# vovach777/llcomp

Hardware: AMD Instinct MI355X
Metric: encode+decode MPix/s on 4K RGB8, bit-exact (higher is better)
Workload: dtype int32

## Files before the change

llcomp_amd/csrc/dec_rows_asm.hpp:

```cpp
#pragma once
#include <cstdint>

namespace llcomp_mi {

#define LD_E0L "v32"
#define LD_E0H "v33"
#define LD_E0 "v[32:33]"
#define LD_E5L "v34"
#define LD_E5H "v35"
#define LD_E5 "v[34:35]"
#define LD_E6L "v36"
#define LD_E6H "v37"
#define LD_E6 "v[36:37]"
#define LD_E7L "v38"
#define LD_E7H "v39"
#define LD_E7 "v[38:39]"
#define LD_E1L "v40"
#define LD_E1H "v41"
#define LD_E1 "v[40:41]"
#define LD_E2L "v42"
#define LD_E2H "v43"
#define LD_E2 "v[42:43]"
#define LD_E3L "v44"
#define LD_E3H "v45"
#define LD_E3 "v[44:45]"
#define LD_E4L "v48"
#define LD_E4H "v49"
#define LD_E4 "v[48:49]"
#define LD_PROD "v50"
#define LD_R1 "v51"
#define LD_DIFF "v52"
#define LD_OFF "v52"
#define LD_EX "v32"
#define LD_W "v33"
#define LD_RUN "v40"
#define LD_NX "v41"
#define LD_T "v42"
#define LD_SX "s[56:57]"
#define LD_SA "s[58:59]"
#define LD_SW "s[60:61]"
#define LD_SP "s[62:63]"
#define LD_S5 "s[64:65]"
#define LD_SU "s[66:67]"
#define LD_SD "s[68:69]"
#define LD_S1L "s[68:69]"
#define LD_SM "s[70:71]"
#define LD_S1 "s70"
#define LD_S2 "s71"

#define LD_SPLIT(EL)                                                                                                       \
    "v_mul_u32_u24_sdwa " LD_PROD ", " EL ", %[range] dst_sel:DWORD dst_unused:UNUSED_PAD src0_sel:BYTE_1 src1_sel:DWORD\n\t" \
    "v_lshrrev_b32_e32 " LD_R1 ", 8, " LD_PROD "\n\t"                                                                      \
    "v_sub_u32_e32 %[range], %[range], " LD_R1 "\n\t"
#define LD_SPLIT_IN(EL)                                                                                                       \
    "v_mul_u32_u24_sdwa " LD_PROD ", " EL ", %[range_in] dst_sel:DWORD dst_unused:UNUSED_PAD src0_sel:BYTE_1 src1_sel:DWORD\n\t" \
    "v_lshrrev_b32_e32 " LD_R1 ", 8, " LD_PROD "\n\t"                                                                      \
    "v_sub_u32_e32 %[range], %[range_in], " LD_R1 "\n\t"
#define LD_REFILL(N)                                         \
    "v_cmp_gt_u32_e32 vcc, %[c100], %[range]\n\t"            \
    "s_and_saveexec_b64 " LD_SW ", vcc\n\t"                  \
    "s_cbranch_execz .Lrf" N "_%=\n\t"                       \
    "v_lshlrev_b32_e32 %[range], 8, %[range]\n\t"            \
    "v_perm_b32 %[low], %[low], %[w32], %[sel]\n\t"          \
    "v_lshrrev_b32_e32 %[w32], 8, %[w32]\n"                   \
    ".Lrf" N "_%=:\n\t"                                      \
    "s_mov_b64 exec, " LD_SW "\n\t"
#define LD_REFILL_R1(N)                                           \
    "v_cmp_gt_u32_e32 vcc, %[c100], " LD_R1 "\n\t"                \
    "s_and_saveexec_b64 " LD_SW ", vcc\n\t"                       \
    "s_cbranch_execz .Lrf" N "_%=\n\t"                            \
    "v_and_b32_e32 %[range], 0xffffff00, " LD_PROD "\n\t"         \
    "v_perm_b32 %[low], %[low], %[w32], %[sel]\n\t"               \
    "v_lshrrev_b32_e32 %[w32], 8, %[w32]\n"                        \
    ".Lrf" N "_%=:\n\t"                                           \
    "s_mov_b64 exec, " LD_SW "\n\t"
#define LD_UNARY(EL, EH, OFS, N, SAVE)                                      \
    LD_SPLIT(EL)                                                            \
    "v_sub_co_u32_e32 %[low], vcc, %[low], %[range]\n\t"                    \
    "ds_write_b16_d16_hi %[bank], " EL " offset:" OFS "\n\t"                \
    "s_andn2_b64 exec, exec, vcc\n\t"                                       \
    SAVE                                                                    \
    "s_cbranch_execz .Lx_done_%=\n\t"                                       \
    "ds_write_b16_d16_hi %[bank], " EH " offset:" OFS "\n\t"                \
    "v_add_u32_e32 " LD_EX ", 1, " LD_EX "\n\t"                                     \
    "v_mov_b32_e32 %[range], " LD_R1 "\n\t"                                 \
    LD_REFILL_R1(N)
#define LD_FETCH_REST                                         \
    "v_lshrrev_b32_e32 " LD_E1L ", 16, %[w0]\n\t"             \
    "v_and_b32_e32 " LD_E2L ", 0xffff, %[w1]\n\t"             \
    "v_lshrrev_b32_e32 " LD_E3L ", 16, %[w1]\n\t"             \
    "v_and_b32_e32 " LD_E4L ", 0xffff, %[w2]\n\t"             \
    "ds_read_b64 " LD_E1 ", " LD_E1L "\n\t"                   \
    "ds_read_b64 " LD_E2 ", " LD_E2L "\n\t"                   \
    "ds_read_b64 " LD_E3 ", " LD_E3L "\n\t"                   \
    "ds_read_b64 " LD_E4 ", " LD_E4L "\n\t"                   \
    "v_lshrrev_b32_e32 " LD_E5L ", 16, %[w2]\n\t"             \
    "v_and_b32_e32 " LD_E6L ", 0xffff, %[w3]\n\t"             \
    "v_lshrrev_b32_e32 " LD_E7L ", 16, %[w3]\n\t"             \
    "ds_read_b64 " LD_E5 ", " LD_E5L "\n\t"                   \
    "ds_read_b64 " LD_E6 ", " LD_E6L "\n\t"                   \
    "ds_read_b64 " LD_E7 ", " LD_E7L "\n\t"

__device__ __forceinline__ void dec_rows_sample_asm(uint32_t low_in, uint32_t range_in, unsigned long long win_in, uint32_t& low,
                                                    uint32_t& range, unsigned long long& win, uint32_t w0, uint32_t w1, uint32_t w2,
                                                    uint32_t w3, uint32_t bank, uint32_t& hot, uint32_t& value, uint32_t& w32) {
    asm volatile(
        "s_mov_b64 " LD_SX ", exec\n\t"
        "v_and_b32_e32 %[w32], 0xffffff, %[winl_in]\n\t"
        "v_or_b32_e32 %[w32], 0x1000000, %[w32]\n\t"
        "v_and_b32_e32 " LD_OFF ", 0xffff, %[w0]\n\t"
        "ds_read_b64 " LD_E0 ", " LD_OFF "\n\t"
        "v_mov_b32_e32 %[value], 0\n\t"
        "s_cmp_lg_u32 %[hot], 0\n\t"
        "s_cbranch_scc0 .Lcold_%=\n\t"
        LD_FETCH_REST
        "s_waitcnt lgkmcnt(7)\n\t"
        "s_branch .Lzero_%=\n"
        ".Lcold_%=:\n\t"
        "s_waitcnt lgkmcnt(0)\n"
        ".Lzero_%=:\n\t"
        LD_SPLIT_IN(LD_E0L)
        "v_sub_co_u32_e32 %[low], vcc, %[low_in], %[range]\n\t"
        "ds_write_b16_d16_hi %[bank], " LD_E0L "\n\t"
        "s_and_b64 " LD_SA ", exec, vcc\n\t"
        "v_cndmask_b32_e32 %[low], %[low], %[low_in], vcc\n\t"
        "s_andn2_b64 exec, exec, vcc\n\t"
        "s_cbranch_execz .Lz1_%=\n\t"
        "v_mov_b32_e32 %[range], " LD_R1 "\n\t"
        "ds_write_b16_d16_hi %[bank], " LD_E0H "\n"
        ".Lz1_%=:\n\t"
        "s_mov_b64 exec, " LD_SX "\n\t"
        LD_REFILL("0")
        "s_and_b64 exec, " LD_SA ", " LD_SA "\n\t"
        "s_cbranch_execz .Ldone_%=\n\t"
        "s_cmp_lg_u32 %[hot], 0\n\t"
        "s_cbranch_scc1 .Lhave_%=\n\t"
        LD_FETCH_REST
        ".Lhave_%=:\n\t"
        "v_mov_b32_e32 " LD_EX ", 0\n\t"
        "v_mov_b32_e32 " LD_W ", 1\n\t"
        "s_waitcnt lgkmcnt(0)\n\t"
        "s_mov_b64 " LD_SM ", 0\n\t"
        LD_UNARY(LD_E1L, LD_E1H, "2", "1", "s_mov_b64 " LD_S1L ", exec\n\t")
        LD_UNARY(LD_E2L, LD_E2H, "256", "2", "s_mov_b64 " LD_SM ", exec\n\t")
        LD_UNARY(LD_E3L, LD_E3H, "258", "3", "")
        "s_mov_b64 " LD_SU ", exec\n\t"
        ".p2align 6\n"
        ".Lu_%=:\n\t"
        "s_waitcnt lgkmcnt(0)\n\t"
        LD_SPLIT(LD_E4L)
        "v_sub_co_u32_e32 %[low], vcc, %[low], %[range]\n\t"
        "s_andn2_b64 exec, exec, vcc\n\t"
        "s_cbranch_execz .Lu_done_%=\n\t"
        "v_lshrrev_b32_e32 " LD_OFF ", 16, " LD_E4H "\n\t"
        "ds_read_b64 " LD_E4 ", " LD_OFF "\n\t"
        "v_add_u32_e32 " LD_EX ", 1, " LD_EX "\n\t"
        "v_mov_b32_e32 %[range], " LD_R1 "\n\t"
        LD_REFILL_R1("4")
        "s_branch .Lu_%=\n"
        ".Lu_done_%=:\n\t"
        "s_mov_b64 exec, " LD_SU "\n\t"
        "ds_write_b16_d16_hi %[bank], " LD_E4L " offset:512\n"
        ".Lx_done_%=:\n\t"
        "s_mov_b64 exec, " LD_SA "\n\t"
        "v_add_u32_e32 %[low], %[low], %[range]\n\t"
        LD_REFILL("5")
        "v_cmp_lt_u32_e32 vcc, 31, " LD_EX "\n\t"
        "s_cbranch_vccz .Lexok_%=\n\t"
        "s_and_saveexec_b64 " LD_SP ", vcc\n\t"
        "v_mov_b32_e32 %[w32], 0\n\t"
        "s_andn2_b64 exec, " LD_SP ", exec\n\t"
        "s_cbranch_execz .Ldone_%=\n"
        ".Lexok_%=:\n\t"
        "s_mov_b64 " LD_S5 ", exec\n\t"
        "s_and_b64 exec, exec, " LD_S1L "\n\t"
        "s_cbranch_execz .Lvalue_%=\n\t"
        "s_mov_b64 " LD_SU ", exec\n\t"
        LD_SPLIT(LD_E5L)
        "v_sub_co_u32_e32 " LD_DIFF ", vcc, %[low], %[range]\n\t"
        "ds_write_b16_d16_hi %[bank], " LD_E5L " offset:514\n\t"
        "s_andn2_b64 " LD_SP ", exec, vcc\n\t"
        "v_addc_co_u32_e32 " LD_W ", vcc, " LD_W ", " LD_W ", vcc\n\t"
        "v_mov_b32_e32 " LD_RUN ", 0\n\t"
        "s_and_b64 exec, " LD_SP ", " LD_SP "\n\t"
        "s_cbranch_execz .Lp5_%=\n\t"
        "v_mov_b32_e32 %[low], " LD_DIFF "\n\t"
        "v_mov_b32_e32 %[range], " LD_R1 "\n\t"
        "ds_write_b16_d16_hi %[bank], " LD_E5H " offset:514\n"
        ".Lp5_%=:\n\t"
        "s_mov_b64 exec, " LD_SU "\n\t"
        LD_REFILL("6")
        "v_add_u32_e32 " LD_T ", -1, " LD_EX "\n\t"
        "s_and_b64 exec, exec, " LD_SM "\n\t"
        "s_cbranch_execz .Lm_skip_%=\n\t"
        "s_mov_b64 " LD_SP ", exec\n\t"
        "v_add_u32_e32 " LD_NX ", -2, " LD_EX "\n\t"
        "v_lshrrev_b32_e32 " LD_RUN ", " LD_NX ", %[sentv]\n\t"
        ".p2align 6\n"
        ".Lm_%=:\n\t"
        "s_waitcnt lgkmcnt(0)\n\t"
        LD_SPLIT(LD_E6L)
        "v_sub_co_u32_e32 " LD_DIFF ", vcc, %[low], %[range]\n\t"
        "s_nop 1\n\t"
        "v_cndmask_b32_e32 %[range], " LD_R1 ", %[range], vcc\n\t"
        "v_cndmask_b32_e32 %[low], " LD_DIFF ", %[low], vcc\n\t"
        "v_cndmask_b32_e32 " LD_NX ", " LD_E6H ", " LD_E6L ", vcc\n\t"
        "v_addc_co_u32_e32 " LD_RUN ", vcc, " LD_RUN ", " LD_RUN ", vcc\n\t"
        "s_mov_b64 " LD_SD ", vcc\n\t"
        "v_lshrrev_b32_e32 " LD_OFF ", 16, " LD_NX "\n\t"
        "ds_read_b64 " LD_E6 ", " LD_OFF "\n\t"
        "v_cmp_gt_u32_e32 vcc, %[c100], %[range]\n\t"
        "s_and_saveexec_b64 " LD_SW ", vcc\n\t"
        "s_cbranch_execz .Lmr_%=\n\t"
        "v_lshlrev_b32_e32 %[range], 8, %[range]\n\t"
        "v_perm_b32 %[low], %[low], %[w32], %[sel]\n\t"
        "v_lshrrev_b32_e32 %[w32], 8, %[w32]\n"
        ".Lmr_%=:\n\t"
        "s_andn2_b64 exec, " LD_SW ", " LD_SD "\n\t"
        "s_cbranch_execnz .Lm_%=\n\t"
        "s_mov_b64 exec, " LD_SP "\n\t"
        "ds_write_b16_d16_hi %[bank], " LD_NX " offset:768\n"
        ".Lm_skip_%=:\n\t"
        "s_mov_b64 exec, " LD_SU "\n\t"
        "v_lshlrev_b32_e32 " LD_W ", " LD_T ", " LD_W "\n\t"
        "v_or_b32_e32 " LD_W ", " LD_W ", " LD_RUN "\n"
        ".Lvalue_%=:\n\t"
        "s_mov_b64 exec, " LD_S5 "\n\t"
        "v_lshlrev_b32_e64 " LD_T ", " LD_EX ", 1\n\t"
        "v_add_u32_e32 " LD_T ", -1, " LD_T "\n\t"
        "v_xor_b32_e32 %[value], " LD_W ", " LD_T "\n\t"
        LD_SPLIT(LD_E7L)
        "v_sub_co_u32_e32 " LD_DIFF ", vcc, %[low], %[range]\n\t"
        "ds_write_b16_d16_hi %[bank], " LD_E7L " offset:770\n\t"
        "s_andn2_b64 exec, exec, vcc\n\t"
        "s_cbranch_execz .Lp7_%=\n\t"
        "v_mov_b32_e32 %[low], " LD_DIFF "\n\t"
        "v_mov_b32_e32 %[range], " LD_R1 "\n\t"
        "ds_write_b16_d16_hi %[bank], " LD_E7H " offset:770\n\t"
        "v_sub_u32_e32 %[value], 0, %[value]\n"
        ".Lp7_%=:\n\t"
        "s_mov_b64 exec, " LD_S5 "\n\t"
        LD_REFILL("7")
        ".Ldone_%=:\n\t"
        "s_mov_b64 exec, " LD_SX "\n\t"
        "v_ffbh_u32_e32 " LD_DIFF ", %[w32]\n\t"
        "v_add_u32_e32 " LD_DIFF ", -7, " LD_DIFF "\n\t"
        "v_lshrrev_b64 %[win], " LD_DIFF ", %[win_in]\n\t"
        "s_bcnt1_i32_b64 " LD_S1 ", " LD_SA "\n\t"
        "s_bcnt1_i32_b64 " LD_S2 ", " LD_SX "\n\t"
        "s_lshl_b32 " LD_S1 ", " LD_S1 ", 1\n\t"
        "s_cmp_ge_u32 " LD_S1 ", " LD_S2 "\n\t"
        "s_cselect_b32 %[hot], 1, 0\n\t"
        "s_mov_b64 exec, " LD_SX "\n\t"
        : [low] "=&v"(low), [range] "=&v"(range), [win] "=&v"(win), [hot] "+s"(hot), [value] "=&v"(value), [w32] "=&v"(w32)
        : [low_in] "v"(low_in), [range_in] "v"(range_in), [win_in] "v"(win_in), [winl_in] "v"(uint32_t(win_in)), [w0] "v"(w0), [w1] "v"(w1), [w2] "v"(w2), [w3] "v"(w3), [bank] "v"(bank), [c100] "s"(0x100u), [sel] "s"(0x06050400u),
          [sentv] "v"(0x80000000u)
        : "vcc", "scc", "memory", "v32", "v33", "v34", "v35", "v36", "v37", "v38", "v39", "v40", "v41", "v42", "v43", "v44", "v45",
          "v48", "v49", "v50", "v51", "v52", "s56", "s57", "s58", "s59", "s60", "s61", "s62", "s63", "s64", "s65", "s66",
          "s67", "s68", "s69", "s70", "s71");
}

}
```

llcomp_amd/csrc/slice_kernels.hip:

```cpp
#include <algorithm>
#include <type_traits>

#include "device_common.hpp"
#include "kernels.hpp"

#ifndef LLMI_ASM_ENC
#define LLMI_ASM_ENC 1
#endif
#if LLMI_ASM_ENC
#include "enc_rows_asm.hpp"
#endif
#ifndef LLMI_ASM_DEC
#define LLMI_ASM_DEC 1
#endif
#if LLMI_ASM_DEC
#include "dec_rows_asm.hpp"
#endif

namespace llcomp_mi {

namespace {

#ifdef LLMI_CLOCK_PROBE
constexpr uint32_t kProbeSlots = 1u << 15;
// ... 839 lines not shown
        "v_cndmask_b32_e32 %[nx], %[hi], %[lo], vcc\n\t"
        "v_addc_co_u32_e32 %[w], vcc, %[w], %[w], vcc"
        : [diff] "=&v"(diff), [range] "=&v"(d.range), [low] "+v"(d.low), [nx] "=&v"(nx), [w] "+v"(w)
        : [r0] "v"(r0), [r1] "v"(r1), [lo] "v"(uint32_t(cur)), [hi] "v"(uint32_t(cur >> 32))
        : "vcc");
    if (d.range < 0x100) {
        d.range <<= 8;
        d.low = (d.low << 8) | (uint32_t(d.win) & 0xFF);
        d.win = window_next(d.win);
    }
    return nx;
}
template <int SLOT, bool CHECKED, bool INLDS>
__device__ __forceinline__ bool dec_once(RangeDec& d, Bank& bank, const Entries& E) {
    const entry_t en = E.get<SLOT>();
    const bool bit = dec_core<CHECKED>(d, prob_of(en));
    dec_put_state<SLOT, INLDS>(bank, successor(en, bit));
    return bit;
}
template <bool ALL, bool CHECKED, bool INLDS>
__device__ __forceinline__ bool dec_residual(RangeDec& d, Bank& bank, const entry_t* tab, uint32_t& out) {
    Entries E;
    dec_fetch_slot0<INLDS>(E, bank, tab);
    if (ALL) dec_fetch_rest<INLDS>(E, bank, tab);
    if (dec_once<0, CHECKED, INLDS>(d, bank, E)) {
        out = 0;
        return true;
    }
    if (!ALL) dec_fetch_rest<INLDS>(E, bank, tab);
    int ex = 0;
    bool ok = true;
    if (dec_once<1, CHECKED, INLDS>(d, bank, E)) {
        ex = 1;
        if (dec_once<2, CHECKED, INLDS>(d, bank, E)) {
            ex = 2;
            if (dec_once<3, CHECKED, INLDS>(d, bank, E)) {
                entry_t cur = E.e4;
                int n = 0;
                for (;;) {
                    if (CHECKED && d.win <= 1) dec_append_drained(d);
                    const uint32_t r1 = __umul24(d.range, prob_of(cur)) >> 8;
                    d.range -= r1;
                    ++n;
                    asm volatile("" : "+v"(n));
                    uint32_t diff;
                    if (__builtin_usub_overflow(d.low, d.range, &diff)) break;
                    d.low = diff;
                    d.range = r1;
                    if (CHECKED && n > 29) break;
                    cur = entry_at(tab, uint32_t(cur >> 32));
                    dec_refill(d);
                }
                dec_refill(d);
                ex = 2 + n;
                if (ex > 31) ok = false;
                const uint32_t nx = uint32_t(cur);
                dec_put_state<4, INLDS>(bank, nx);
            }
        }
    }
    if (!ok) return false;
    uint32_t w = 1;
    const uint32_t ones = (1u << ex) - 1;
    if (ex > 0) {
        w += w + uint32_t(!dec_once<5, CHECKED, INLDS>(d, bank, E));
        if (ex > 1) {
            entry_t cur = E.e6;
            uint32_t nx;
            uint32_t limit = ones + 1;
            asm volatile("" : "+v"(limit));
            do {
                nx = dec_step_acc<CHECKED>(d, prob_of(cur), cur, w);
                cur = entry_at(tab, nx);
            } while (w < limit);
            dec_put_state<6, INLDS>(bank, nx);
        }
    }
    uint32_t v = w ^ ones;
    if (dec_once<7, CHECKED, INLDS>(d, bank, E)) v = 0u - v;
    out = v;
    return true;
}

template <bool INLDS>
__device__ __forceinline__ bool dec_sample(RangeDec& d, Bank& bank, const entry_t* tab, uint32_t& hot, bool replay_always,
                                           uint32_t& v) {
#if LLMI_ASM_DEC
    if constexpr (INLDS) {
        uint32_t low, range, left;
        unsigned long long win;
        dec_rows_sample_asm(d.low, d.range, d.win, low, range, win, bank.w[0], bank.w[1], bank.w[2], bank.w[3], lds_address(bank.lds), hot, v,
                            left);
        if (__builtin_expect(left == 0 || replay_always, 0)) {
            ++d.replays;
            reinterpret_cast<uint32_t*>(bank.lds)[0] = bank.w[0];
            reinterpret_cast<uint32_t*>(bank.lds)[64] = bank.w[1];
            reinterpret_cast<uint32_t*>(bank.lds)[128] = bank.w[2];
            reinterpret_cast<uint32_t*>(bank.lds)[192] = bank.w[3];
            asm("v_mov_b32_e32 %0, %3\n\tv_mov_b32_e32 %1, %4\n\tv_mov_b64_e32 %2, %5"
                : "+v"(low), "+v"(range), "+v"(win)
                : "v"(d.low), "v"(d.range), "v"(d.win));
            d.low = low;
            d.range = range;
            d.win = win;
            return dec_residual<false, true, true>(d, bank, tab, v);
        }
        d.low = low;
        d.range = range;
        d.win = win;
        return true;
    } else
#endif
    {
        const uint32_t s_low = d.low, s_range = d.range, s_b0 = bank.w[0], s_b1 = bank.w[1], s_b2 = bank.w[2], s_b3 = bank.w[3];
        const unsigned long long s_win = d.win;
        bool ok = hot ? dec_residual<true, false, INLDS>(d, bank, tab, v) : dec_residual<false, false, INLDS>(d, bank, tab, v);
        hot = 2 * __popcll(__ballot(v != 0)) >= __popcll(__ballot(true));
        if (__builtin_expect(!ok || d.win == 0 || replay_always, 0)) {
            ++d.replays;
            d.low = s_low; d.range = s_range; d.win = s_win;
            bank.w[0] = s_b0; bank.w[1] = s_b1;
            if constexpr (INLDS) {
                bank.w[2] = s_b2; bank.w[3] = s_b3;
                reinterpret_cast<uint32_t*>(bank.lds)[0] = s_b0;
                reinterpret_cast<uint32_t*>(bank.lds)[64] = s_b1;
                reinterpret_cast<uint32_t*>(bank.lds)[128] = s_b2;
                reinterpret_cast<uint32_t*>(bank.lds)[192] = s_b3;
            }
            ok = dec_residual<false, true, INLDS>(d, bank, tab, v);
        }
        return ok;
    }
}

constexpr uint32_t bank_cache_lds_bytes(int log2_entries) { return log2_entries ? (64u * 9u) << log2_entries : 0u; }
template <int NCH, bool ROWS, bool LDSTAB = false, int CACHE = 0, bool SMALL = false>
__global__ __launch_bounds__(64, ROWS && NCH == 1 ? 8 : 1) void k_decode_slices(const Geometry g, const uint32_t lpw_and_flags,
                                                      const uint8_t* __restrict__ units,
                                                      const uint32_t* __restrict__ slice_len,
                                                      uint64_t* __restrict__ states, int16_t* __restrict__ rec,
                                                      uint32_t* status, const uint64_t gpat,
                                                      unsigned long long* __restrict__ counters) {
    __shared__ entry_t tab[128];
    __shared__ uint32_t rowbank[ROWS ? kWideBankWords : 1];
    __shared__ int8_t quant_lut[ROWS ? 1 : 512];
    if constexpr (!ROWS) {
        for (uint32_t i = threadIdx.x; i < 256; i += blockDim.x) {
            quant_lut[i] = int8_t(quant11(int(i) - 128));
            quant_lut[256 + i] = int8_t(quant5(int(i) - 128));
        }
    }
    static_assert(CACHE == 0 || (!ROWS && !LDSTAB && NCH != 0), "the bank cache belongs to the 2-D kernels with tables in HBM");
    static_assert(!SMALL || ROWS, "the model is a template flag of the 1-row-slice kernels only");
    static_assert(CACHE == 0 || ((kContexts - 1) >> CACHE) < 0xFF, "bank cache: a context's tag would alias the empty marker");
    __shared__ uint32_t wave_sums[CACHE != 0 ? 2 : 1];
    clear_lds_states<LDSTAB>();
    if constexpr (CACHE != 0) {
        uint32_t* tg = reinterpret_cast<uint32_t*>(dyn_lds + (512u << CACHE));
        for (uint32_t i = threadIdx.x; i < (16u << CACHE); i += blockDim.x) tg[i] = 0xFFFFFFFFu;
        if (threadIdx.x < 2) wave_sums[threadIdx.x] = 0;
    }
    load_table(tab);
    const uint32_t lpw = lpw_and_flags & 0xFF;
    const bool replay_always = (lpw_and_flags >> 8) & 1;
    [[maybe_unused]] const bool small_model = (g.flags & kGeoSmallModel) != 0;
    const uint32_t id = blockIdx.x * lpw + threadIdx.x;
    if (threadIdx.x >= lpw || id >= g.n_slices) return;
    const SliceRect r = slice_rect(g, id);
    RangeDec d;
    const uint32_t len = min(slice_len[id], g.slice_cap - 16);
    const uint32_t grp = __builtin_amdgcn_readfirstlane(id >> g.lane_shift);
    const uint32_t lane_in_group = id & ((1u << g.lane_shift) - 1);
    dec_open(d, reinterpret_cast<const uint32_t*>(units) + ((size_t(grp) * (g.slice_cap >> 2)) << g.lane_shift), lane_in_group,
             g.lane_shift, len);

    int16_t* p0 = rec + lane_order_index(g, id, 0);
    const ptrdiff_t GW = ptrdiff_t(1) << g.lane_shift;
    int16_t* const gbase = rec + ((size_t(grp) * g.slice_samples) << g.lane_shift);
    uint32_t hot = 0;
    LLMI_PROBE_START();

    if constexpr (ROWS) {
        for (uint32_t k = 0; k < 12; ++k) rowbank[k * 64 + threadIdx.x] = lds_address(tab) * 0x00010001u;
        int l[NCH], L[NCH];
#pragma unroll
        for (int k = 0; k < NCH; ++k) l[k] = L[k] = 128;
        int held_val = 0;
        uint32_t store_ofs = lane_in_group * 2, step_ofs = 2u << g.lane_shift;
        asm volatile("" : "+v"(step_ofs));
        uint8_t* const bank0 = reinterpret_cast<uint8_t*>(rowbank) + threadIdx.x * 4;
        bool bad = false;
        auto pixel = [&](auto model, auto start) {
            constexpr int MODEL = decltype(model)::value;
            constexpr bool START = decltype(start)::value;
#pragma unroll
            for (int k = 0; k < NCH; ++k) {
                if (window_low(d)) dec_append(d);
                if (!(START && k == 0)) {
                    asm volatile("global_store_short %0, %1, %2" : : "v"(store_ofs), "v"(held_val), "s"(gbase) : "memory");
                    store_ofs += step_ofs;
                }
                const int lv = l[k];
                uint32_t sg = 0, bofs = 0;
                if constexpr (MODEL != kModelSmall) {
                    const int dq = L[k] - lv;
                    sg = uint32_t(dq >> 31);
                    asm volatile("" : "+v"(sg));
                    const uint32_t aq = (uint32_t(dq) ^ sg) - sg;
                    uint32_t o1 = ((aq + 0x7FFFFFFFu) >> 21) & 0x400u, o2 = ((aq + 0x7FFFFFFCu) >> 21) & 0x400u;
                    asm volatile("" : "+v"(o1), "+v"(o2));
                    bofs = o1 + o2;
                }
                uint32_t* bp = reinterpret_cast<uint32_t*>(bank0 + bofs);
                Bank bank{{bp[0], bp[64], bp[128], bp[192]}, reinterpret_cast<uint8_t*>(bp)};
                uint32_t v = 0;
                if (!dec_sample<true>(d, bank, tab, hot, replay_always, v)) bad = true;
                if constexpr (MODEL != kModelSmall) v = (v ^ sg) - sg;
                const int val = int(int16_t(uint32_t(lv) + v));
                held_val = val;
                L[k] = START ? val : lv;
                l[k] = val;
            }
        };
        const uint32_t sw0 = __builtin_amdgcn_readfirstlane(r.sw);
        const uint32_t n_bulk = __builtin_amdgcn_ballot_w64(r.sw != sw0) == 0 ? sw0 : 0;
        uint32_t x = 1;
        pixel(no_model, std::true_type{});
        constexpr std::integral_constant<int, SMALL ? kModelSmall : kModelLarge> model{};
        if constexpr (NCH == 1) {
            for (; x + 1 < n_bulk; x += 2) {
                pixel(model, std::false_type{});
                pixel(model, std::false_type{});
            }
        } else {
            for (; x < n_bulk; ++x) pixel(model, std::false_type{});
        }
        for (; x < r.sw; ++x) pixel(model, std::false_type{});
        if (bad) atomicOr(status, kStBadExponent);
        asm volatile("global_store_short %0, %1, %2" : : "v"(store_ofs), "v"(held_val), "s"(gbase) : "memory");
        publish_count(counters, kCtrDecReplays, d.replays);
    } else {
        uint64_t* banks;
        uint32_t bsh;
        if constexpr (LDSTAB) {
            banks = reinterpret_cast<uint64_t*>(dyn_lds);
            bsh = 0;
        } else {
            banks = states + ((size_t(id >> g.lane_shift) * kContexts) << g.lane_shift) + (id & ((1u << g.lane_shift) - 1));
            bsh = g.lane_shift;
        }
        if constexpr (NCH == 0) {
            const uint32_t nch = g.nch;
            const ptrdiff_t px_step = ptrdiff_t(nch) * GW, up = ptrdiff_t(r.sw) * px_step;
            for (uint32_t y = 0; y < r.sh; ++y) {
                for (uint32_t x = 0; x < r.sw; ++x) {
                    for (uint32_t k = 0; k < nch; ++k) {
                        int16_t* q = p0 + ptrdiff_t(y) * up + ptrdiff_t(x) * px_step + ptrdiff_t(k) * GW;
                        if (window_low(d)) dec_append(d);
                        const Hood n = apply_borders(x > 0 ? q[-px_step] : 0, x > 1 ? q[-2 * px_step] : 0, y > 0 ? q[-up] : 0,
                                                     (y > 0 && x > 0) ? q[-up - px_step] : 0, (y > 0 && x + 1 < r.sw) ? q[-up + px_step] : 0,
                                                     y > 1 ? q[-2 * up] : 0, x, y, r.sw);
                        int ctx = context_hash(n, small_model);
                        const bool neg = ctx < 0;
                        if (neg) ctx = -ctx;
                        const uint64_t b64 = bank_fresh<LDSTAB>(banks[size_t(ctx) << bsh], gpat);
                        Bank bank{{uint32_t(b64), uint32_t(b64 >> 32)}, nullptr};
                        uint32_t v;
                        if (!dec_sample<false>(d, bank, tab, hot, replay_always, v)) {
                            atomicOr(status, kStBadExponent);
                            return;
                        }
                                banks[size_t(ctx) << bsh] = bank_tagged<LDSTAB>(uint64_t(bank.w[0]) | (uint64_t(bank.w[1]) << 32), gpat);
                        if (neg) v = 0u - v;
                        *q = int16_t(uint32_t(predict(n)) + v);
                    }
                }
            }
            publish_count(counters, kCtrDecReplays, d.replays);
        } else {
        const ptrdiff_t up = ptrdiff_t(r.sw) * NCH * GW;
        uint32_t held_ctx = ~0u;
        uint64_t held_bank = 0;
        [[maybe_unused]] uint64_t wb_bank = 0;
        [[maybe_unused]] uint64_t* wb_ptr = nullptr;
        [[maybe_unused]] bool use_cache = CACHE != 0;
        [[maybe_unused]] uint32_t my_miss = 0, my_lookups = 0, my_wb = 0, miss_mark = 0, look_mark = 0;
        LLMI_PARTS_DECL();
        LLMI_PARTS_START();
        for (uint32_t y = 0; y < r.sh; ++y) {
            if constexpr (CACHE != 0) {
                const uint32_t yu = __builtin_amdgcn_readfirstlane(y);
                if (use_cache && yu >= 4 && (yu & 3) == 0) {
                    __hip_atomic_fetch_add(&wave_sums[0], my_miss - miss_mark, __ATOMIC_RELAXED, __HIP_MEMORY_SCOPE_WORKGROUP);
                    __hip_atomic_fetch_add(&wave_sums[1], my_lookups - look_mark, __ATOMIC_RELAXED, __HIP_MEMORY_SCOPE_WORKGROUP);
                    miss_mark = my_miss;
                    look_mark = my_lookups;
                    const uint32_t n_miss = __builtin_amdgcn_readfirstlane(__hip_atomic_load(&wave_sums[0], __ATOMIC_RELAXED, __HIP_MEMORY_SCOPE_WORKGROUP));
                    const uint32_t n_seen = __builtin_amdgcn_readfirstlane(__hip_atomic_load(&wave_sums[1], __ATOMIC_RELAXED, __HIP_MEMORY_SCOPE_WORKGROUP));
                    __hip_atomic_store(&wave_sums[0], 0u, __ATOMIC_RELAXED, __HIP_MEMORY_SCOPE_WORKGROUP);
                    __hip_atomic_store(&wave_sums[1], 0u, __ATOMIC_RELAXED, __HIP_MEMORY_SCOPE_WORKGROUP);
                    if (yu >= 8 && n_miss * 8 > n_seen * 7) {
// ... 262 lines not shown
```

Baseline: 30760.

## Compute next-sample context bank inside decode asm to shorten dependency chain

For 1–2 channel row decoders, the inline-asm sample decoder now reads the bank words itself from an LDS address and, while decoding, derives the next sample's context bank offset from the decoded exponent. This takes the bank-offset arithmetic (which needed the previously decoded value) off the critical path between consecutive samples. The speculative offset assumes the exponent stays within a bound and no int16 wrap happens. When that does not hold, the code restores the bank words and replays the sample through the C++ decoder. It adds extra LDS reads and more complex control flow, and when speculation misses it pays the replay cost.

```diff
diff --git a/llcomp_amd/csrc/dec_rows_asm.hpp b/llcomp_amd/csrc/dec_rows_asm.hpp
--- a/llcomp_amd/csrc/dec_rows_asm.hpp
+++ b/llcomp_amd/csrc/dec_rows_asm.hpp
@@ -85,179 +85,37 @@
     "v_add_u32_e32 " LD_EX ", 1, " LD_EX "\n\t"                                     \
     "v_mov_b32_e32 %[range], " LD_R1 "\n\t"                                 \
     LD_REFILL_R1(N)
+#define LD_FETCH_ADDR                                             \
+    "ds_read_u16 " LD_E0L ", %[bank]\n\t"                         \
+    "ds_read_u16 " LD_E1L ", %[bank] offset:2\n\t"                \
+    "ds_read_u16 " LD_E2L ", %[bank] offset:256\n\t"              \
+    "ds_read_u16 " LD_E3L ", %[bank] offset:258\n\t"              \
+    "ds_read_u16 " LD_E4L ", %[bank] offset:512\n\t"              \
+    "ds_read_u16 " LD_E5L ", %[bank] offset:514\n\t"              \
+    "ds_read_u16 " LD_E6L ", %[bank] offset:768\n\t"              \
+    "ds_read_u16 " LD_E7L ", %[bank] offset:770\n\t"              \
+    "ds_read_b32 %[w0], %[bank]\n\t"                              \
+    "ds_read_b32 %[w1], %[bank] offset:256\n\t"                   \
+    "ds_read_b32 %[w2], %[bank] offset:512\n\t"                   \
+    "ds_read_b32 %[w3], %[bank] offset:768\n\t"
 #define LD_FETCH_REST                                         \
-    "v_lshrrev_b32_e32 " LD_E1L ", 16, %[w0]\n\t"             \
-    "v_and_b32_e32 " LD_E2L ", 0xffff, %[w1]\n\t"             \
-    "v_lshrrev_b32_e32 " LD_E3L ", 16, %[w1]\n\t"             \
-    "v_and_b32_e32 " LD_E4L ", 0xffff, %[w2]\n\t"             \
     "ds_read_b64 " LD_E1 ", " LD_E1L "\n\t"                   \
     "ds_read_b64 " LD_E2 ", " LD_E2L "\n\t"                   \
     "ds_read_b64 " LD_E3 ", " LD_E3L "\n\t"                   \
     "ds_read_b64 " LD_E4 ", " LD_E4L "\n\t"                   \
-    "v_lshrrev_b32_e32 " LD_E5L ", 16, %[w2]\n\t"             \
-    "v_and_b32_e32 " LD_E6L ", 0xffff, %[w3]\n\t"             \
-    "v_lshrrev_b32_e32 " LD_E7L ", 16, %[w3]\n\t"             \
     "ds_read_b64 " LD_E5 ", " LD_E5L "\n\t"                   \
     "ds_read_b64 " LD_E6 ", " LD_E6L "\n\t"                   \
     "ds_read_b64 " LD_E7 ", " LD_E7L "\n\t"
+#define LD_RUN_BIN                                            \
+    LD_SPLIT(LD_E4L)                                          \
+    "v_sub_co_u32_e32 %[low], vcc, %[low], %[range]\n\t"      \
+    "s_andn2_b64 exec, exec, vcc\n\t"
 
-__device__ __forceinline__ void dec_rows_sample_asm(uint32_t low_in, uint32_t range_in, unsigned long long win_in, uint32_t& low,
-                                                    uint32_t& range, unsigned long long& win, uint32_t w0, uint32_t w1, uint32_t w2,
-                                                    uint32_t w3, uint32_t bank, uint32_t& hot, uint32_t& value, uint32_t& w32) {
-    asm volatile(
-        "s_mov_b64 " LD_SX ", exec\n\t"
-        "v_and_b32_e32 %[w32], 0xffffff, %[winl_in]\n\t"
-        "v_or_b32_e32 %[w32], 0x1000000, %[w32]\n\t"
-        "v_and_b32_e32 " LD_OFF ", 0xffff, %[w0]\n\t"
-        "ds_read_b64 " LD_E0 ", " LD_OFF "\n\t"
-        "v_mov_b32_e32 %[value], 0\n\t"
-        "s_cmp_lg_u32 %[hot], 0\n\t"
-        "s_cbranch_scc0 .Lcold_%=\n\t"
-        LD_FETCH_REST
-        "s_waitcnt lgkmcnt(7)\n\t"
-        "s_branch .Lzero_%=\n"
-        ".Lcold_%=:\n\t"
-        "s_waitcnt lgkmcnt(0)\n"
-        ".Lzero_%=:\n\t"
-        LD_SPLIT_IN(LD_E0L)
-        "v_sub_co_u32_e32 %[low], vcc, %[low_in], %[range]\n\t"
-        "ds_write_b16_d16_hi %[bank], " LD_E0L "\n\t"
-        "s_and_b64 " LD_SA ", exec, vcc\n\t"
-        "v_cndmask_b32_e32 %[low], %[low], %[low_in], vcc\n\t"
-        "s_andn2_b64 exec, exec, vcc\n\t"
-        "s_cbranch_execz .Lz1_%=\n\t"
-        "v_mov_b32_e32 %[range], " LD_R1 "\n\t"
-        "ds_write_b16_d16_hi %[bank], " LD_E0H "\n"
-        ".Lz1_%=:\n\t"
-        "s_mov_b64 exec, " LD_SX "\n\t"
-        LD_REFILL("0")
-        "s_and_b64 exec, " LD_SA ", " LD_SA "\n\t"
-        "s_cbranch_execz .Ldone_%=\n\t"
-        "s_cmp_lg_u32 %[hot], 0\n\t"
-        "s_cbranch_scc1 .Lhave_%=\n\t"
-        LD_FETCH_REST
-        ".Lhave_%=:\n\t"
-        "v_mov_b32_e32 " LD_EX ", 0\n\t"
-        "v_mov_b32_e32 " LD_W ", 1\n\t"
-        "s_waitcnt lgkmcnt(0)\n\t"
-        "s_mov_b64 " LD_SM ", 0\n\t"
-        LD_UNARY(LD_E1L, LD_E1H, "2", "1", "s_mov_b64 " LD_S1L ", exec\n\t")
-        LD_UNARY(LD_E2L, LD_E2H, "256", "2", "s_mov_b64 " LD_SM ", exec\n\t")
-        LD_UNARY(LD_E3L, LD_E3H, "258", "3", "")
-        "s_mov_b64 " LD_SU ", exec\n\t"
-        ".p2align 6\n"
-        ".Lu_%=:\n\t"
-        "s_waitcnt lgkmcnt(0)\n\t"
-        LD_SPLIT(LD_E4L)
-        "v_sub_co_u32_e32 %[low], vcc, %[low], %[range]\n\t"
-        "s_andn2_b64 exec, exec, vcc\n\t"
-        "s_cbranch_execz .Lu_done_%=\n\t"
-        "v_lshrrev_b32_e32 " LD_OFF ", 16, " LD_E4H "\n\t"
-        "ds_read_b64 " LD_E4 ", " LD_OFF "\n\t"
-        "v_add_u32_e32 " LD_EX ", 1, " LD_EX "\n\t"
-        "v_mov_b32_e32 %[range], " LD_R1 "\n\t"
-        LD_REFILL_R1("4")
-        "s_branch .Lu_%=\n"
-        ".Lu_done_%=:\n\t"
-        "s_mov_b64 exec, " LD_SU "\n\t"
-        "ds_write_b16_d16_hi %[bank], " LD_E4L " offset:512\n"
-        ".Lx_done_%=:\n\t"
-        "s_mov_b64 exec, " LD_SA "\n\t"
-        "v_add_u32_e32 %[low], %[low], %[range]\n\t"
-        LD_REFILL("5")
-        "v_cmp_lt_u32_e32 vcc, 31, " LD_EX "\n\t"
-        "s_cbranch_vccz .Lexok_%=\n\t"
-        "s_and_saveexec_b64 " LD_SP ", vcc\n\t"
-        "v_mov_b32_e32 %[w32], 0\n\t"
-        "s_andn2_b64 exec, " LD_SP ", exec\n\t"
-        "s_cbranch_execz .Ldone_%=\n"
-        ".Lexok_%=:\n\t"
-        "s_mov_b64 " LD_S5 ", exec\n\t"
-        "s_and_b64 exec, exec, " LD_S1L "\n\t"
-        "s_cbranch_execz .Lvalue_%=\n\t"
-        "s_mov_b64 " LD_SU ", exec\n\t"
-        LD_SPLIT(LD_E5L)
-        "v_sub_co_u32_e32 " LD_DIFF ", vcc, %[low], %[range]\n\t"
-        "ds_write_b16_d16_hi %[bank], " LD_E5L " offset:514\n\t"
-        "s_andn2_b64 " LD_SP ", exec, vcc\n\t"
-        "v_addc_co_u32_e32 " LD_W ", vcc, " LD_W ", " LD_W ", vcc\n\t"
-        "v_mov_b32_e32 " LD_RUN ", 0\n\t"
-        "s_and_b64 exec, " LD_SP ", " LD_SP "\n\t"
-        "s_cbranch_execz .Lp5_%=\n\t"
-        "v_mov_b32_e32 %[low], " LD_DIFF "\n\t"
-        "v_mov_b32_e32 %[range], " LD_R1 "\n\t"
-        "ds_write_b16_d16_hi %[bank], " LD_E5H " offset:514\n"
-        ".Lp5_%=:\n\t"
-        "s_mov_b64 exec, " LD_SU "\n\t"
-        LD_REFILL("6")
-        "v_add_u32_e32 " LD_T ", -1, " LD_EX "\n\t"
-        "s_and_b64 exec, exec, " LD_SM "\n\t"
-        "s_cbranch_execz .Lm_skip_%=\n\t"
-        "s_mov_b64 " LD_SP ", exec\n\t"
-        "v_add_u32_e32 " LD_NX ", -2, " LD_EX "\n\t"
-        "v_lshrrev_b32_e32 " LD_RUN ", " LD_NX ", %[sentv]\n\t"
-        ".p2align 6\n"
-        ".Lm_%=:\n\t"
-        "s_waitcnt lgkmcnt(0)\n\t"
-        LD_SPLIT(LD_E6L)
-        "v_sub_co_u32_e32 " LD_DIFF ", vcc, %[low], %[range]\n\t"
-        "s_nop 1\n\t"
-        "v_cndmask_b32_e32 %[range], " LD_R1 ", %[range], vcc\n\t"
-        "v_cndmask_b32_e32 %[low], " LD_DIFF ", %[low], vcc\n\t"
-        "v_cndmask_b32_e32 " LD_NX ", " LD_E6H ", " LD_E6L ", vcc\n\t"
-        "v_addc_co_u32_e32 " LD_RUN ", vcc, " LD_RUN ", " LD_RUN ", vcc\n\t"
-        "s_mov_b64 " LD_SD ", vcc\n\t"
-        "v_lshrrev_b32_e32 " LD_OFF ", 16, " LD_NX "\n\t"
-        "ds_read_b64 " LD_E6 ", " LD_OFF "\n\t"
-        "v_cmp_gt_u32_e32 vcc, %[c100], %[range]\n\t"
-        "s_and_saveexec_b64 " LD_SW ", vcc\n\t"
-        "s_cbranch_execz .Lmr_%=\n\t"
-        "v_lshlrev_b32_e32 %[range], 8, %[range]\n\t"
-        "v_perm_b32 %[low], %[low], %[w32], %[sel]\n\t"
-        "v_lshrrev_b32_e32 %[w32], 8, %[w32]\n"
-        ".Lmr_%=:\n\t"
-        "s_andn2_b64 exec, " LD_SW ", " LD_SD "\n\t"
-        "s_cbranch_execnz .Lm_%=\n\t"
-        "s_mov_b64 exec, " LD_SP "\n\t"
-        "ds_write_b16_d16_hi %[bank], " LD_NX " offset:768\n"
-        ".Lm_skip_%=:\n\t"
-        "s_mov_b64 exec, " LD_SU "\n\t"
-        "v_lshlrev_b32_e32 " LD_W ", " LD_T ", " LD_W "\n\t"
-        "v_or_b32_e32 " LD_W ", " LD_W ", " LD_RUN "\n"
-        ".Lvalue_%=:\n\t"
-        "s_mov_b64 exec, " LD_S5 "\n\t"
-        "v_lshlrev_b32_e64 " LD_T ", " LD_EX ", 1\n\t"
-        "v_add_u32_e32 " LD_T ", -1, " LD_T "\n\t"
-        "v_xor_b32_e32 %[value], " LD_W ", " LD_T "\n\t"
-        LD_SPLIT(LD_E7L)
-        "v_sub_co_u32_e32 " LD_DIFF ", vcc, %[low], %[range]\n\t"
-        "ds_write_b16_d16_hi %[bank], " LD_E7L " offset:770\n\t"
-        "s_andn2_b64 exec, exec, vcc\n\t"
-        "s_cbranch_execz .Lp7_%=\n\t"
-        "v_mov_b32_e32 %[low], " LD_DIFF "\n\t"
-        "v_mov_b32_e32 %[range], " LD_R1 "\n\t"
-        "ds_write_b16_d16_hi %[bank], " LD_E7H " offset:770\n\t"
-        "v_sub_u32_e32 %[value], 0, %[value]\n"
-        ".Lp7_%=:\n\t"
-        "s_mov_b64 exec, " LD_S5 "\n\t"
-        LD_REFILL("7")
-        ".Ldone_%=:\n\t"
-        "s_mov_b64 exec, " LD_SX "\n\t"
-        "v_ffbh_u32_e32 " LD_DIFF ", %[w32]\n\t"
-        "v_add_u32_e32 " LD_DIFF ", -7, " LD_DIFF "\n\t"
-        "v_lshrrev_b64 %[win], " LD_DIFF ", %[win_in]\n\t"
-        "s_bcnt1_i32_b64 " LD_S1 ", " LD_SA "\n\t"
-        "s_bcnt1_i32_b64 " LD_S2 ", " LD_SX "\n\t"
-        "s_lshl_b32 " LD_S1 ", " LD_S1 ", 1\n\t"
-        "s_cmp_ge_u32 " LD_S1 ", " LD_S2 "\n\t"
-        "s_cselect_b32 %[hot], 1, 0\n\t"
-        "s_mov_b64 exec, " LD_SX "\n\t"
-        : [low] "=&v"(low), [range] "=&v"(range), [win] "=&v"(win), [hot] "+s"(hot), [value] "=&v"(value), [w32] "=&v"(w32)
-        : [low_in] "v"(low_in), [range_in] "v"(range_in), [win_in] "v"(win_in), [winl_in] "v"(uint32_t(win_in)), [w0] "v"(w0), [w1] "v"(w1), [w2] "v"(w2), [w3] "v"(w3), [bank] "v"(bank), [c100] "s"(0x100u), [sel] "s"(0x06050400u),
-          [sentv] "v"(0x80000000u)
-        : "vcc", "scc", "memory", "v32", "v33", "v34", "v35", "v36", "v37", "v38", "v39", "v40", "v41", "v42", "v43", "v44", "v45",
-          "v48", "v49", "v50", "v51", "v52", "s56", "s57", "s58", "s59", "s60", "s61", "s62", "s63", "s64", "s65", "s66",
-          "s67", "s68", "s69", "s70", "s71");
-}
+#define LD_NEXT 0
+#include "dec_sample_asm.inc"
+#undef LD_NEXT
+#define LD_NEXT 1
+#include "dec_sample_asm.inc"
+#undef LD_NEXT
 
 }
diff --git a/llcomp_amd/csrc/dec_sample_asm.inc b/llcomp_amd/csrc/dec_sample_asm.inc
--- /dev/null
+++ b/llcomp_amd/csrc/dec_sample_asm.inc
@@ -0,0 +1,188 @@
+#if LD_NEXT
+#define LD_IF_NEXT(...) __VA_ARGS__
+#define LD_EXMAX "14"
+#else
+#define LD_IF_NEXT(...)
+#define LD_EXMAX "31"
+#endif
+#if LD_NEXT
+__device__ __forceinline__ void dec_rows_sample_next_asm(uint32_t low_in, uint32_t range_in, unsigned long long win_in, uint32_t& low,
+                                                         uint32_t& range, unsigned long long& win, uint32_t& w0, uint32_t& w1,
+                                                         uint32_t& w2, uint32_t& w3, uint32_t bank, uint32_t bank0, uint32_t& next,
+                                                         uint32_t& hot, uint32_t& value, uint32_t& w32) {
+#else
+__device__ __forceinline__ void dec_rows_sample_asm(uint32_t low_in, uint32_t range_in, unsigned long long win_in, uint32_t& low,
+                                                    uint32_t& range, unsigned long long& win, uint32_t& w0, uint32_t& w1, uint32_t& w2,
+                                                    uint32_t& w3, uint32_t bank, uint32_t& hot, uint32_t& value, uint32_t& w32) {
+#endif
+    asm volatile(
+        "s_mov_b64 " LD_SX ", exec\n\t"
+        "s_waitcnt lgkmcnt(0)\n\t"
+        LD_FETCH_ADDR
+        "v_and_b32_e32 %[w32], 0xffffff, %[winl_in]\n\t"
+        "v_or_b32_e32 %[w32], 0x1000000, %[w32]\n\t"
+        "v_mov_b32_e32 %[value], 0\n\t"
+        LD_IF_NEXT("v_mov_b32_e32 %[next], %[bank0]\n\t")
+        "s_cmp_lg_u32 %[hot], 0\n\t"
+        "s_waitcnt lgkmcnt(11)\n\t"
+        "ds_read_b64 " LD_E0 ", " LD_E0L "\n\t"
+        "s_cbranch_scc0 .Lcold_%=\n\t"
+        "s_waitcnt lgkmcnt(5)\n\t"
+        LD_FETCH_REST
+        "s_waitcnt lgkmcnt(7)\n\t"
+        "s_branch .Lzero_%=\n"
+        ".Lcold_%=:\n\t"
+        "s_waitcnt lgkmcnt(0)\n"
+        ".Lzero_%=:\n\t"
+        LD_SPLIT_IN(LD_E0L)
+        "v_sub_co_u32_e32 %[low], vcc, %[low_in], %[range]\n\t"
+        "ds_write_b16_d16_hi %[bank], " LD_E0L "\n\t"
+        "s_and_b64 " LD_SA ", exec, vcc\n\t"
+        "v_cndmask_b32_e32 %[low], %[low], %[low_in], vcc\n\t"
+        "s_andn2_b64 exec, exec, vcc\n\t"
+        "s_cbranch_execz .Lz1_%=\n\t"
+        "v_mov_b32_e32 %[range], " LD_R1 "\n\t"
+        "ds_write_b16_d16_hi %[bank], " LD_E0H "\n"
+        ".Lz1_%=:\n\t"
+        "s_mov_b64 exec, " LD_SX "\n\t"
+        LD_REFILL("0")
+        "s_and_b64 exec, " LD_SA ", " LD_SA "\n\t"
+        "s_cbranch_execz .Ldone_%=\n\t"
+        "s_cmp_lg_u32 %[hot], 0\n\t"
+        "s_cbranch_scc1 .Lhave_%=\n\t"
+        LD_FETCH_REST
+        ".Lhave_%=:\n\t"
+        "v_mov_b32_e32 " LD_EX ", 0\n\t"
+        "v_mov_b32_e32 " LD_W ", 1\n\t"
+        "s_waitcnt lgkmcnt(0)\n\t"
+        "s_mov_b64 " LD_SM ", 0\n\t"
+        LD_UNARY(LD_E1L, LD_E1H, "2", "1", "s_mov_b64 " LD_S1L ", exec\n\t")
+        LD_UNARY(LD_E2L, LD_E2H, "256", "2", "s_mov_b64 " LD_SM ", exec\n\t")
+        LD_UNARY(LD_E3L, LD_E3H, "258", "3", "")
+        "s_mov_b64 " LD_SU ", exec\n\t"
+        LD_RUN_BIN
+        "s_cbranch_execz .Lu_done_%=\n\t"
+        ".p2align 6\n"
+        ".Lu_%=:\n\t"
+        "v_lshrrev_b32_e32 " LD_OFF ", 16, " LD_E4H "\n\t"
+        "ds_read_b64 " LD_E4 ", " LD_OFF "\n\t"
+        "v_add_u32_e32 " LD_EX ", 1, " LD_EX "\n\t"
+        "v_mov_b32_e32 %[range], " LD_R1 "\n\t"
+        LD_REFILL_R1("4")
+        "s_waitcnt lgkmcnt(0)\n\t"
+        LD_RUN_BIN
+        "s_cbranch_execnz .Lu_%=\n"
+        ".Lu_done_%=:\n\t"
+        "s_mov_b64 exec, " LD_SU "\n\t"
+        "ds_write_b16_d16_hi %[bank], " LD_E4L " offset:512\n"
+        ".Lx_done_%=:\n\t"
+        "s_mov_b64 exec, " LD_SA "\n\t"
+        LD_IF_NEXT("v_add_u32_e32 %[next], 0x400, %[next]\n\t")
+        "v_add_u32_e32 %[low], %[low], %[range]\n\t"
+        LD_REFILL("5")
+        "v_cmp_lt_u32_e32 vcc, " LD_EXMAX ", " LD_EX "\n\t"
+        "s_cbranch_vccz .Lexok_%=\n\t"
+        "s_and_saveexec_b64 " LD_SP ", vcc\n\t"
+        "v_mov_b32_e32 %[w32], 0\n\t"
+        "s_andn2_b64 exec, " LD_SP ", exec\n\t"
+        "s_cbranch_execz .Ldone_%=\n"
+        ".Lexok_%=:\n\t"
+        "s_mov_b64 " LD_S5 ", exec\n\t"
+        "s_and_b64 exec, exec, " LD_S1L "\n\t"
+        "s_cbranch_execz .Lvalue_%=\n\t"
+        "s_mov_b64 " LD_SU ", exec\n\t"
+        LD_SPLIT(LD_E5L)
+        "v_sub_co_u32_e32 " LD_DIFF ", vcc, %[low], %[range]\n\t"
+        "ds_write_b16_d16_hi %[bank], " LD_E5L " offset:514\n\t"
+        "s_andn2_b64 " LD_SP ", exec, vcc\n\t"
+        "v_addc_co_u32_e32 " LD_W ", vcc, " LD_W ", " LD_W ", vcc\n\t"
+        "v_mov_b32_e32 " LD_RUN ", 0\n\t"
+        "s_and_b64 exec, " LD_SP ", " LD_SP "\n\t"
+        "s_cbranch_execz .Lp5_%=\n\t"
+        "v_mov_b32_e32 %[low], " LD_DIFF "\n\t"
+        "v_mov_b32_e32 %[range], " LD_R1 "\n\t"
+        "ds_write_b16_d16_hi %[bank], " LD_E5H " offset:514\n"
+        ".Lp5_%=:\n\t"
+        "s_mov_b64 exec, " LD_SU "\n\t"
+        LD_REFILL("6")
+        "v_add_u32_e32 " LD_T ", -1, " LD_EX "\n\t"
+        "s_and_b64 exec, exec, " LD_SM "\n\t"
+        "s_cbranch_execz .Lm_skip_%=\n\t"
+        "s_mov_b64 " LD_SP ", exec\n\t"
+        "v_add_u32_e32 " LD_NX ", -2, " LD_EX "\n\t"
+        LD_IF_NEXT("v_add_u32_e32 %[next], 0x400, %[next]\n\t")
+        "v_lshrrev_b32_e32 " LD_RUN ", " LD_NX ", %[sentv]\n\t"
+        ".p2align 6\n"
+        ".Lm_%=:\n\t"
+        "s_waitcnt lgkmcnt(0)\n\t"
+        LD_SPLIT(LD_E6L)
+        "v_sub_co_u32_e32 " LD_DIFF ", vcc, %[low], %[range]\n\t"
+        "s_nop 1\n\t"
+        "v_cndmask_b32_e32 %[range], " LD_R1 ", %[range], vcc\n\t"
+        "v_cndmask_b32_e32 %[low], " LD_DIFF ", %[low], vcc\n\t"
+        "v_cndmask_b32_e32 " LD_NX ", " LD_E6H ", " LD_E6L ", vcc\n\t"
+        "v_addc_co_u32_e32 " LD_RUN ", vcc, " LD_RUN ", " LD_RUN ", vcc\n\t"
+        "s_mov_b64 " LD_SD ", vcc\n\t"
+        "v_lshrrev_b32_e32 " LD_OFF ", 16, " LD_NX "\n\t"
+        "ds_read_b64 " LD_E6 ", " LD_OFF "\n\t"
+        "v_cmp_gt_u32_e32 vcc, %[c100], %[range]\n\t"
+        "s_and_saveexec_b64 " LD_SW ", vcc\n\t"
+        "s_cbranch_execz .Lmr_%=\n\t"
+        "v_lshlrev_b32_e32 %[range], 8, %[range]\n\t"
+        "v_perm_b32 %[low], %[low], %[w32], %[sel]\n\t"
+        "v_lshrrev_b32_e32 %[w32], 8, %[w32]\n"
+        ".Lmr_%=:\n\t"
+        "s_andn2_b64 exec, " LD_SW ", " LD_SD "\n\t"
+        "s_cbranch_execnz .Lm_%=\n\t"
+        "s_mov_b64 exec, " LD_SP "\n\t"
+        "ds_write_b16_d16_hi %[bank], " LD_NX " offset:768\n"
+        ".Lm_skip_%=:\n\t"
+        "s_mov_b64 exec, " LD_SU "\n\t"
+        "v_lshlrev_b32_e32 " LD_W ", " LD_T ", " LD_W "\n\t"
+        "v_or_b32_e32 " LD_W ", " LD_W ", " LD_RUN "\n"
+        ".Lvalue_%=:\n\t"
+        "s_mov_b64 exec, " LD_S5 "\n\t"
+        "v_lshlrev_b32_e64 " LD_T ", " LD_EX ", 1\n\t"
+        "v_add_u32_e32 " LD_T ", -1, " LD_T "\n\t"
+        "v_xor_b32_e32 %[value], " LD_W ", " LD_T "\n\t"
+        LD_SPLIT(LD_E7L)
+        "v_sub_co_u32_e32 " LD_DIFF ", vcc, %[low], %[range]\n\t"
+        "ds_write_b16_d16_hi %[bank], " LD_E7L " offset:770\n\t"
+        "s_andn2_b64 exec, exec, vcc\n\t"
+        "s_cbranch_execz .Lp7_%=\n\t"
+        "v_mov_b32_e32 %[low], " LD_DIFF "\n\t"
+        "v_mov_b32_e32 %[range], " LD_R1 "\n\t"
+        "ds_write_b16_d16_hi %[bank], " LD_E7H " offset:770\n\t"
+        "v_sub_u32_e32 %[value], 0, %[value]\n"
+        ".Lp7_%=:\n\t"
+        "s_mov_b64 exec, " LD_S5 "\n\t"
+        LD_REFILL("7")
+        ".Ldone_%=:\n\t"
+        "s_mov_b64 exec, " LD_SX "\n\t"
+        "s_waitcnt lgkmcnt(0)\n\t"
+        "v_ffbh_u32_e32 " LD_DIFF ", %[w32]\n\t"
+        "v_add_u32_e32 " LD_DIFF ", -7, " LD_DIFF "\n\t"
+        "v_lshrrev_b64 %[win], " LD_DIFF ", %[win_in]\n\t"
+        "s_bcnt1_i32_b64 " LD_S1 ", " LD_SA "\n\t"
+        "s_bcnt1_i32_b64 " LD_S2 ", " LD_SX "\n\t"
+        "s_lshl_b32 " LD_S1 ", " LD_S1 ", 1\n\t"
+        "s_cmp_ge_u32 " LD_S1 ", " LD_S2 "\n\t"
+        "s_cselect_b32 %[hot], 1, 0\n\t"
+        "s_mov_b64 exec, " LD_SX "\n\t"
+        : [low] "=&v"(low), [range] "=&v"(range), [win] "=&v"(win), [hot] "+s"(hot), [value] "=&v"(value), [w32] "=&v"(w32),
+          [w0] "=&v"(w0), [w1] "=&v"(w1), [w2] "=&v"(w2), [w3] "=&v"(w3)
+#if LD_NEXT
+          , [next] "=&v"(next)
+#endif
+        : [low_in] "v"(low_in), [range_in] "v"(range_in), [win_in] "v"(win_in), [winl_in] "v"(uint32_t(win_in)), [bank] "v"(bank),
+#if LD_NEXT
+          [bank0] "v"(bank0),
+#endif
+          [c100] "s"(0x100u), [sel] "s"(0x06050400u), [sentv] "v"(0x80000000u)
+        : "vcc", "scc", "memory", "v32", "v33", "v34", "v35", "v36", "v37", "v38", "v39", "v40", "v41", "v42", "v43", "v44", "v45",
+          "v48", "v49", "v50", "v51", "v52", "s56", "s57", "s58", "s59", "s60", "s61", "s62", "s63", "s64", "s65", "s66",
+          "s67", "s68", "s69", "s70", "s71");
+}
+
+#undef LD_IF_NEXT
+#undef LD_EXMAX
diff --git a/llcomp_amd/csrc/slice_kernels.hip b/llcomp_amd/csrc/slice_kernels.hip
--- a/llcomp_amd/csrc/slice_kernels.hip
+++ b/llcomp_amd/csrc/slice_kernels.hip
@@ -945,6 +945,50 @@
     return true;
 }
 
+__device__ __forceinline__ uint32_t rows_bank_offset(int dq, uint32_t sg) {
+    const uint32_t aq = (uint32_t(dq) ^ sg) - sg;
+    uint32_t o1 = ((aq + 0x7FFFFFFFu) >> 21) & 0x400u, o2 = ((aq + 0x7FFFFFFCu) >> 21) & 0x400u;
+    asm volatile("" : "+v"(o1), "+v"(o2));
+    return o1 + o2;
+}
+#if LLMI_ASM_DEC
+__device__ __forceinline__ bool dec_sample_next(RangeDec& d, const entry_t* tab, uint8_t* bank0, uint32_t cur, uint32_t& next, int dq, int lv,
+                                                uint32_t sg, uint32_t& wrapped, uint32_t& hot, bool replay_always, uint32_t& v) {
+    uint32_t low, range, left, w0, w1, w2, w3;
+    unsigned long long win;
+    dec_rows_sample_next_asm(d.low, d.range, d.win, low, range, win, w0, w1, w2, w3, cur, lds_address(bank0), next, hot, v, left);
+    if (__builtin_expect(left <= wrapped || replay_always, 0)) {
+        ++d.replays;
+        auto* touched = reinterpret_cast<__attribute__((address_space(3))) uint32_t*>(uintptr_t(cur));
+        touched[0] = w0;
+        touched[64] = w1;
+        touched[128] = w2;
+        touched[192] = w3;
+        uint32_t* bp = reinterpret_cast<uint32_t*>(bank0 + rows_bank_offset(dq, sg));
+        Bank bank{{bp[0], bp[64], bp[128], bp[192]}, reinterpret_cast<uint8_t*>(bp)};
+        asm("v_mov_b32_e32 %0, %3\n\tv_mov_b32_e32 %1, %4\n\tv_mov_b64_e32 %2, %5"
+            : "+v"(low), "+v"(range), "+v"(win)
+            : "v"(d.low), "v"(d.range), "v"(d.win));
+        d.low = low;
+        d.range = range;
+        d.win = win;
+        const bool ok = dec_residual<false, true, true>(d, bank, tab, v);
+        uint32_t vr = v;
+        asm volatile("" : "+v"(vr));
+        const uint32_t sum = uint32_t(lv) + ((vr ^ sg) - sg);
+        const int stored = int(int16_t(sum));
+        if (sum != uint32_t(stored)) wrapped = ~0u;
+        const int dn = lv - stored;
+        next = lds_address(bank0) + rows_bank_offset(dn, uint32_t(dn >> 31));
+        return ok;
+    }
+    d.low = low;
+    d.range = range;
+    d.win = win;
+    return true;
+}
+#endif
+
 template <bool INLDS>
 __device__ __forceinline__ bool dec_sample(RangeDec& d, Bank& bank, const entry_t* tab, uint32_t& hot, bool replay_always,
                                            uint32_t& v) {
@@ -997,6 +1041,8 @@
 }
 
 constexpr uint32_t bank_cache_lds_bytes(int log2_entries) { return log2_entries ? (64u * 9u) << log2_entries : 0u; }
+template <int NCH>
+constexpr bool kRowsDecNextBank = NCH <= 2;
 template <int NCH, bool ROWS, bool LDSTAB = false, int CACHE = 0, bool SMALL = false>
 __global__ __launch_bounds__(64, ROWS && NCH == 1 ? 8 : 1) void k_decode_slices(const Geometry g, const uint32_t lpw_and_flags,
                                                       const uint8_t* __restrict__ units,
@@ -1053,9 +1099,13 @@
         asm volatile("" : "+v"(step_ofs));
         uint8_t* const bank0 = reinterpret_cast<uint8_t*>(rowbank) + threadIdx.x * 4;
         bool bad = false;
+        [[maybe_unused]] uint32_t next_bank[NCH], wrapped = 0;
+#pragma unroll
+        for (int k = 0; k < NCH; ++k) next_bank[k] = lds_address(bank0);
         auto pixel = [&](auto model, auto start) {
             constexpr int MODEL = decltype(model)::value;
             constexpr bool START = decltype(start)::value;
+            constexpr bool NEXT = LLMI_ASM_DEC != 0 && MODEL != kModelSmall && kRowsDecNextBank<NCH>;
 #pragma unroll
             for (int k = 0; k < NCH; ++k) {
                 if (window_low(d)) dec_append(d);
@@ -1065,21 +1115,29 @@
                 }
                 const int lv = l[k];
                 uint32_t sg = 0, bofs = 0;
+                [[maybe_unused]] int dq = 0;
                 if constexpr (MODEL != kModelSmall) {
-                    const int dq = L[k] - lv;
+                    dq = L[k] - lv;
+                    if constexpr (NEXT) asm volatile("" : "+v"(dq));
                     sg = uint32_t(dq >> 31);
                     asm volatile("" : "+v"(sg));
-                    const uint32_t aq = (uint32_t(dq) ^ sg) - sg;
-                    uint32_t o1 = ((aq + 0x7FFFFFFFu) >> 21) & 0x400u, o2 = ((aq + 0x7FFFFFFCu) >> 21) & 0x400u;
-                    asm volatile("" : "+v"(o1), "+v"(o2));
-                    bofs = o1 + o2;
+                    if constexpr (!NEXT) bofs = rows_bank_offset(dq, sg);
                 }
-                uint32_t* bp = reinterpret_cast<uint32_t*>(bank0 + bofs);
-                Bank bank{{bp[0], bp[64], bp[128], bp[192]}, reinterpret_cast<uint8_t*>(bp)};
                 uint32_t v = 0;
-                if (!dec_sample<true>(d, bank, tab, hot, replay_always, v)) bad = true;
+#if LLMI_ASM_DEC
+                if constexpr (NEXT) {
+                    if (!dec_sample_next(d, tab, bank0, next_bank[k], next_bank[k], dq, lv, sg, wrapped, hot, replay_always, v)) bad = true;
+                } else
+#endif
+                {
+                    uint32_t* bp = reinterpret_cast<uint32_t*>(bank0 + bofs);
+                    Bank bank{{bp[0], bp[64], bp[128], bp[192]}, reinterpret_cast<uint8_t*>(bp)};
+                    if (!dec_sample<true>(d, bank, tab, hot, replay_always, v)) bad = true;
+                }
                 if constexpr (MODEL != kModelSmall) v = (v ^ sg) - sg;
-                const int val = int(int16_t(uint32_t(lv) + v));
+                const uint32_t sum = uint32_t(lv) + v;
+                const int val = int(int16_t(sum));
+                if constexpr (NEXT) wrapped |= sum ^ uint32_t(val);
                 held_val = val;
                 L[k] = START ? val : lv;
                 l[k] = val;
```

After: 30880, median of 6. Within noise of the previous version (+0.4%).
